# privacy-scaling-explorations/snark-verifier

Hardware: AMD Instinct MI355X
Metric: BN254 G1 MSM points/sec at 2^20 (higher is better)
Workload: dtype i32x9 (254-bit Montgomery Fq as 9 x 29-bit limbs on the integer VALU); 1 GPU; BN254 G1 Pippenger MSM, 2^20 random points/scalars per GPU, inputs resident in HBM, affine result (configs[1]); points_per_gpu=1048576, points_per_kernel_launch=1048576, window_bits=default, msms_in_flight=264

## Files before the change

snark-verifier_amd/csrc/bn254_consts.h:

```cpp
#pragma once
#define SNARKV_CURVE_NAME "bn254"
#define SNARKV_FQ_P_LIMBS { 0xd87cfd47u, 0x3c208c16u, 0x6871ca8du, 0x97816a91u, 0x8181585du, 0xb85045b6u, 0xe131a029u, 0x30644e72u }
#define SNARKV_FQ_P_INV32 0xe4866389u
#define SNARKV_FQ_ONE_MONT { 0xc58f0d9du, 0xd35d438du, 0xf5c70b3du, 0x0a78eb28u, 0x7879462cu, 0x666ea36fu, 0x9a07df2fu, 0x0e0a77c1u }
#define SNARKV_FQ_R2_MONT { 0x538afa89u, 0xf32cfc5bu, 0xd44501fbu, 0xb5e71911u, 0x0a417ff6u, 0x47ab1effu, 0xcab8351fu, 0x06d89f71u }
#define SNARKV_FQ_P_MINUS_2_LIMBS { 0xd87cfd45u, 0x3c208c16u, 0x6871ca8du, 0x97816a91u, 0x8181585du, 0xb85045b6u, 0xe131a029u, 0x30644e72u }
#define SNARKV_G1_B_MONT { 0x50ad28d7u, 0x7a17caa9u, 0xe15521b9u, 0x1f6ac17au, 0x696bd284u, 0x334bea4eu, 0xce179d8eu, 0x2a1f6744u }
#define SNARKV_FR_R_LIMBS { 0xf0000001u, 0x43e1f593u, 0x79b97091u, 0x2833e848u, 0x8181585du, 0xb85045b6u, 0xe131a029u, 0x30644e72u }
#define SNARKV_FQ29_P_LIMBS { 0x187cfd47, 0x010460b6, 0x1c72a34f, 0x02d522d0, 0x1585d978, 0x02db40c0, 0x00a6e141, 0x0e5c2634, 0x0030644e }
#define SNARKV_FQ29_NINV 0x04866389
#define SNARKV_FQ29_ONE_LIMBS { 0x157ccc21, 0x141c2758, 0x185230d3, 0x014c0419, 0x0aa36fb9, 0x1d4240ce, 0x11d54c07, 0x052ac7a8, 0x000dc836 }
#define SNARKV_FQ29_R2_LIMBS { 0x059bac10, 0x0d1503a3, 0x018016b8, 0x10ab0ca8, 0x02632639, 0x02c0169f, 0x169bfd53, 0x11869d4c, 0x002a11a6 }
#define SNARKV_FQ29_M256_IN_LIMBS { 0x13349ca1, 0x1a5d84a8, 0x0a3e5cac, 0x100249e0, 0x12b951e8, 0x0e92d304, 0x14cb95b3, 0x041b9d3d, 0x00058003 }
#define SNARKV_FQ29_M256_OUT_LIMBS { 0x058f0d9d, 0x1aea1c6e, 0x11c2cf74, 0x11d651eb, 0x1462c0a7, 0x11b7bc3c, 0x1cbd99ba, 0x183340fb, 0x000e0a77 }
#define SNARKV_FR29_P_LIMBS { 0x10000001, 0x1f0fac9f, 0x0e5c2450, 0x07d090f3, 0x1585d283, 0x02db40c0, 0x00a6e141, 0x0e5c2634, 0x0030644e }
#define SNARKV_FR29_NINV 0x0fffffff
#define SNARKV_FR29_ONE_LIMBS { 0x0fffff57, 0x1ea70ab4, 0x052c068b, 0x17504f49, 0x0aa8075b, 0x1d4240ce, 0x11d54c07, 0x052ac7a8, 0x000dc836 }
#define SNARKV_FR29_R2_LIMBS { 0x05b69bd4, 0x06170a5a, 0x020cddce, 0x1db6310b, 0x0e54d0ff, 0x1cf855e3, 0x1c15e103, 0x07d09161, 0x000a054a }
#define SNARKV_GLV_BETA29_LIMBS { 0x0a337995, 0x158d1d23, 0x189c9b98, 0x12fa4e45, 0x185faadc, 0x0176f16d, 0x0eed93ba, 0x14291140, 0x000c0afe }
#define SNARKV_GLV_A1 { 0x94d213e3u, 0x89d32568u, 0x00000000u, 0x00000000u }
#define SNARKV_GLV_NEG_B1 { 0x7d4f1128u, 0x8211bbebu, 0xeeb859fcu, 0x6f4d8248u }
#define SNARKV_GLV_A2 { 0x1221250bu, 0x0be4e154u, 0xeeb859fdu, 0x6f4d8248u }
#define SNARKV_GLV_B2 { 0x94d213e3u, 0x89d32568u, 0x00000000u, 0x00000000u }
#define SNARKV_GLV_G1 { 0x6eb9c714u, 0xc7e0b3d7u, 0xd91d232eu, 0x00000002u, 0x00000000u, 0x00000000u }
#define SNARKV_GLV_G2 { 0xa5e38cfbu, 0x391eb18du, 0x7a7bd9d4u, 0xa773d2cfu, 0x4ccef014u, 0x00000002u }
#define BN254_P_LIMBS { 0xd87cfd47u, 0x3c208c16u, 0x6871ca8du, 0x97816a91u, 0x8181585du, 0xb85045b6u, 0xe131a029u, 0x30644e72u }
#define BN254_R_LIMBS { 0xf0000001u, 0x43e1f593u, 0x79b97091u, 0x2833e848u, 0x8181585du, 0xb85045b6u, 0xe131a029u, 0x30644e72u }
#define BN254_P_INV32 0xe4866389u
#define BN254_ONE_MONT { 0xc58f0d9du, 0xd35d438du, 0xf5c70b3du, 0x0a78eb28u, 0x7879462cu, 0x666ea36fu, 0x9a07df2fu, 0x0e0a77c1u }
#define BN254_R2_MONT { 0x538afa89u, 0xf32cfc5bu, 0xd44501fbu, 0xb5e71911u, 0x0a417ff6u, 0x47ab1effu, 0xcab8351fu, 0x06d89f71u }
#define BN254_THREE_MONT { 0x50ad28d7u, 0x7a17caa9u, 0xe15521b9u, 0x1f6ac17au, 0x696bd284u, 0x334bea4eu, 0xce179d8eu, 0x2a1f6744u }
#define BN254_TWIST_B_C0_MONT { 0x77b802a8u, 0x3bf938e3u, 0x3633535du, 0x020b1b27u, 0x49755260u, 0x26b7edf0u, 0x4384a86du, 0x2514c632u }
#define BN254_TWIST_B_C1_MONT { 0xd1dcff67u, 0x38e7ecccu, 0x93ce0d3eu, 0x65f0b37du, 0x22ac00aau, 0xd749d0ddu, 0x4a688d4du, 0x0141b9ceu }
#define BN254_TWIST_3B_C0_MONT { 0xb62e0d6au, 0x3baa927cu, 0xd1b664fdu, 0xd71e7c52u, 0xd95d4664u, 0x03873e63u, 0x082ab8f4u, 0x0e75b5b1u }
#define BN254_TWIST_3B_C1_MONT { 0x7596fe35u, 0xaab7c666u, 0xbb6a27bau, 0x31d21a78u, 0x680401ffu, 0x85dd7297u, 0xdf39a7e9u, 0x03c52d6au }
#define BN254_P_MINUS_2_LIMBS { 0xd87cfd45u, 0x3c208c16u, 0x6871ca8du, 0x97816a91u, 0x8181585du, 0xb85045b6u, 0xe131a029u, 0x30644e72u }
#define BN254_P_PLUS_1_DIV_4_LIMBS { 0xb61f3f52u, 0x4f082305u, 0x5a1c72a3u, 0x65e05aa4u, 0xa0605617u, 0x6e14116du, 0xb84c680au, 0x0c19139cu }
#define BN254_X_U64 0x44e992b44a6909f1ull
#define BN254_ATE_LOOP_LO 0x9d797039be763ba8ull
#define BN254_ATE_LOOP_HI 0x1ull
#define BN254_P29_LIMBS { 0x187cfd47, 0x010460b6, 0x1c72a34f, 0x02d522d0, 0x1585d978, 0x02db40c0, 0x00a6e141, 0x0e5c2634, 0x0030644e }
#define BN254_P29_NINV 0x04866389
#define BN254_ONE29_LIMBS { 0x157ccc21, 0x141c2758, 0x185230d3, 0x014c0419, 0x0aa36fb9, 0x1d4240ce, 0x11d54c07, 0x052ac7a8, 0x000dc836 }
#define BN254_R2_29_LIMBS { 0x059bac10, 0x0d1503a3, 0x018016b8, 0x10ab0ca8, 0x02632639, 0x02c0169f, 0x169bfd53, 0x11869d4c, 0x002a11a6 }
#define BN254_THREE29_LIMBS { 0x00766463, 0x1c54760a, 0x08f6927a, 0x03e40c4d, 0x1fea4f2b, 0x17c6c26a, 0x157fe417, 0x0f8056f9, 0x002958a2 }
#define BN254_FR29_LIMBS { 0x10000001, 0x1f0fac9f, 0x0e5c2450, 0x07d090f3, 0x1585d283, 0x02db40c0, 0x00a6e141, 0x0e5c2634, 0x0030644e }
#define BN254_FR29_NINV 0x0fffffff
#define BN254_FR29_ONE_LIMBS { 0x0fffff57, 0x1ea70ab4, 0x052c068b, 0x17504f49, 0x0aa8075b, 0x1d4240ce, 0x11d54c07, 0x052ac7a8, 0x000dc836 }
#define BN254_FR29_R2_LIMBS { 0x05b69bd4, 0x06170a5a, 0x020cddce, 0x1db6310b, 0x0e54d0ff, 0x1cf855e3, 0x1c15e103, 0x07d09161, 0x000a054a }
#define BN254_FROB_GAMMA_1 { \
  { { 0x33144907u, 0xaf9ba696u, 0x87afb78au, 0xca6b1d73u, 0xf08a2087u, 0x11bded5eu, 0x1a1f3a7cu, 0x02f34d75u }, { 0x4c492d72u, 0xa222ae23u, 0x565de15bu, 0xd00f02a4u, 0x53dfc926u, 0xdc2ff3a2u, 0xb3899551u, 0x10a75716u } }, \
  { { 0x4563ab30u, 0xb5773b10u, 0xa9aa6454u, 0x347f91c8u, 0x242e0991u, 0x7a007127u, 0x118214ecu, 0x1956bcd8u }, { 0xa0aa4757u, 0x6e849f1eu, 0x89f89141u, 0xaa1c7b6du, 0xfae0ca3au, 0xb6e713cdu, 0x4e82ebc3u, 0x26694fbbu } }, \
  { { 0x2936b629u, 0xe4bbdd0cu, 0xe133bacbu, 0xbb30f162u, 0xf9645366u, 0x31a9d1b6u, 0xa500f8ddu, 0x253570beu }, { 0x5ffe77c7u, 0xa1d77ce4u, 0x7826d1dbu, 0x07affd11u, 0xbb7edc6bu, 0x6d16bd27u, 0x85defeccu, 0x2c872002u } }, \
  { { 0x843abe92u, 0x7361d77fu, 0x273411fbu, 0xa5bb2bd3u, 0x4b3e2399u, 0x9c941f31u, 0xbb9fd3ecu, 0x15df9cddu }, { 0x4bd8c949u, 0x5dddfd15u, 0xa4445b60u, 0x62cb29a5u, 0x0c7dd2b9u, 0x37bc870au, 0x3171f0fdu, 0x24830a9du } }, \
  { { 0x41690fe7u, 0xc970692fu, 0x27694b0bu, 0xe2403421u, 0x83c459e8u, 0x32bee66bu, 0x0ab08841u, 0x12aabcedu }, { 0x40aebfa9u, 0x0d485d23u, 0xab2fcc57u, 0x05193418u, 0x8a4910f5u, 0xd3b0a40bu, 0x35d2925au, 0x2f21ebb5u } }, \
}
#define BN254_FROB_GAMMA_2 { \
  { { 0x00fa1bf2u, 0xca8d8005u, 0x68b39769u, 0xf0c5d614u, 0xad0d4418u, 0x0e201271u, 0xbad856e6u, 0x04290f65u }, { 0x00000000u, 0x00000000u, 0x00000000u, 0x00000000u, 0x00000000u, 0x00000000u, 0x00000000u, 0x00000000u } }, \
  { { 0x13e80b9cu, 0x3350c88eu, 0xdb5e56b9u, 0x7dce557cu, 0xb615564au, 0x6001b4b8u, 0x020217e0u, 0x2682e617u }, { 0x00000000u, 0x00000000u, 0x00000000u, 0x00000000u, 0x00000000u, 0x00000000u, 0x00000000u, 0x00000000u } }, \
  { { 0x12edefaau, 0x68c34889u, 0x72aabf4fu, 0x8d087f68u, 0x09081231u, 0x51e1a247u, 0x4729c0fau, 0x2259d6b1u }, { 0x00000000u, 0x00000000u, 0x00000000u, 0x00000000u, 0x00000000u, 0x00000000u, 0x00000000u, 0x00000000u } }, \
  { { 0xd782e155u, 0x71930c11u, 0xffbe3323u, 0xa6bb947cu, 0xd4741444u, 0xaa303344u, 0x26594943u, 0x2c3b3f0du }, { 0x00000000u, 0x00000000u, 0x00000000u, 0x00000000u, 0x00000000u, 0x00000000u, 0x00000000u, 0x00000000u } }, \
  { { 0xc494f1abu, 0x08cfc388u, 0x8d1373d4u, 0x19b31514u, 0xcb6c0213u, 0x584e90fdu, 0xdf2f8849u, 0x09e1685bu }, { 0x00000000u, 0x00000000u, 0x00000000u, 0x00000000u, 0x00000000u, 0x00000000u, 0x00000000u, 0x00000000u } }, \
}
#define BN254_FROB_GAMMA_3 { \
  { { 0x4e46d97du, 0x36531618u, 0xd4c96d9fu, 0x0af7129eu, 0xca1009b5u, 0x659da72fu, 0x83a20d23u, 0x08116d89u }, { 0xc39c1939u, 0xb1df4af7u, 0x8a73bf7fu, 0x3d9f0287u, 0x8caf0ae0u, 0x9b222092u, 0xeff054a6u, 0x26684515u } }, \
  { { 0x16ad6badu, 0xc9af22f7u, 0x4aa662b2u, 0xb311782au, 0xe248c7f4u, 0x19eeaf64u, 0xe3439f82u, 0x20273e77u }, { 0xf7ce93acu, 0xacc02860u, 0x7ba76b4cu, 0x3933d581u, 0x446c8467u, 0x69e6188bu, 0x4417cc55u, 0x0a46036du } }, \
  { { 0xaf46471eu, 0x5764af0au, 0x873e0fc1u, 0xdc50792eu, 0x881d04f6u, 0x86a673ffu, 0x3c30a74cu, 0x0b2eddb4u }, { 0x787e8580u, 0x9a490f32u, 0xf04af8b1u, 0x8fd16d7fu, 0xc6027bf2u, 0x4b39888eu, 0x5b52a15du, 0x03dd2e70u } }, \
  { { 0x7b6762dfu, 0x448a93a5u, 0x28fdeadfu, 0xbfd62df5u, 0x0e9bd47au, 0xd858f5d0u, 0x3476ec58u, 0x06b03d4du }, { 0xbcc936d1u, 0x2b19daf4u, 0x56f4299fu, 0xa1a54e7au, 0x5adeaef1u, 0xb533eee0u, 0x84dda0b2u, 0x170c812bu } }, \
  { { 0x75cf559fu, 0xe0bc4b22u, 0xc154e60fu, 0xc238b945u, 0x929a7d5eu, 0x803982a5u, 0xf7e4a37eu, 0x15ce052du }, { 0xbf3799a7u, 0x2d28efbdu, 0x1ad60773u, 0x9b097e3cu, 0xaf4a535bu, 0x982d4113u, 0xe3056063u, 0x24e18991u } }, \
}
#define BN254_FROB29_GAMMA_1 { \
  { { 0x0a0c2399, 0x1aa2357c, 0x0149b22d, 0x0487bf1b, 0x0b89bb5e, 0x1313c7e1, 0x1d61fdb5, 0x060c56b5, 0x002e0560 }, { 0x1bc6cc33, 0x177dfb71, 0x161dd8ab, 0x0180969d, 0x058d47f5, 0x1ab975b5, 0x01c26a2d, 0x1cd88219, 0x00009b83 } }, \
  { { 0x04a59190, 0x06f504d9, 0x0bf870bb, 0x171ffd5c, 0x1ac4d17d, 0x04be36d5, 0x0bceec27, 0x1a83a513, 0x002492b3 }, { 0x11142ef1, 0x0b31acc7, 0x1d5818bc, 0x180afc17, 0x1a63177e, 0x15765b3b, 0x118f742e, 0x063a509a, 0x00135e4e } }, \
  { { 0x1b1f0678, 0x0373fb06, 0x13170fbd, 0x185d74b7, 0x0241131f, 0x16e18435, 0x1ef3b6ce, 0x01f06f02, 0x001d46bd }, { 0x19a647d5, 0x19fdefab, 0x1d925d1a, 0x0d1f6c5f, 0x08ac6cc5, 0x1fa5621a, 0x134f06fe, 0x09a72816, 0x0015871d } }, \
  { { 0x1081f85e, 0x139a3585, 0x124aed48, 0x034ce260, 0x19e166e5, 0x0b172958, 0x0d2df880, 0x0de46877, 0x00167751 }, { 0x0f616a78, 0x05940429, 0x181bb386, 0x066e257b, 0x00e66254, 0x0c12b5cd, 0x0ef6c029, 0x1c2232e3, 0x0006f9f8 } }, \
  { { 0x07461d8c, 0x0434a6b0, 0x14f8b697, 0x0b0aa80f, 0x118b92df, 0x0471333d, 0x18c6d066, 0x07d8f7b0, 0x0010a3f0 }, { 0x1eb54987, 0x08d56d1e, 0x0c80f1d8, 0x1536f380, 0x06b4b4a7, 0x082bcd3c, 0x19349170, 0x17aea9fc, 0x000817f6 } }, \
}
#define BN254_FROB29_GAMMA_2 { \
// ... 18 lines not shown
```

snark-verifier_amd/csrc/gen_consts.py:

```python
#!/usr/bin/env python3
import sys

P = 0x30644E72E131A029B85045B68181585D97816A916871CA8D3C208C16D87CFD47
R = 0x30644E72E131A029B85045B68181585D2833E84879B9709143E1F593F0000001
X = 4965661367192848881
MONT_R = 1 << 256


def generic_section(p, r, b, name):
    def lim(v):
        return ", ".join("0x%08xu" % ((v >> (32 * i)) & 0xFFFFFFFF) for i in range(8))

    def lim29(v):
        return ", ".join("0x%08x" % ((v >> (29 * i)) & ((1 << 29) - 1)) for i in range(9))

    r29 = 1 << 261
    print("// ---- field / group layer constants of %s: base field p, scalar field r, y^2 = x^3 + %d" % (name, b))
    print("#define SNARKV_CURVE_NAME \"%s\"" % name)
    print("#define SNARKV_FQ_P_LIMBS { %s }" % lim(p))
    print("#define SNARKV_FQ_P_INV32 0x%08xu  // -p^-1 mod 2^32" % ((-pow(p, -1, 1 << 32)) % (1 << 32)))
    print("#define SNARKV_FQ_ONE_MONT { %s }  // 2^256 mod p" % lim(MONT_R % p))
    print("#define SNARKV_FQ_R2_MONT { %s }  // 2^512 mod p" % lim(MONT_R * MONT_R % p))
    print("#define SNARKV_FQ_P_MINUS_2_LIMBS { %s }" % lim(p - 2))
    print("#define SNARKV_G1_B_MONT { %s }  // b * 2^256 mod p" % lim(b * MONT_R % p))
# ... 21 lines not shown
    def add(a, b):
        if a is None:
            return b
        if b is None:
            return a
        if a[0] == b[0]:
            if (a[1] + b[1]) % p == 0:
                return None
            l = 3 * a[0] * a[0] * pow(2 * a[1], -1, p) % p
        else:
            l = (b[1] - a[1]) * pow(b[0] - a[0], -1, p) % p
        x = (l * l - a[0] - b[0]) % p
        return (x, (l * (a[0] - x) - a[1]) % p)

    acc = None
    for bit in bin(k)[2:]:
        acc = add(acc, acc)
        if bit == "1":
            acc = add(acc, pt)
    return acc


def _glv_lattice(n, lam):
    import math

    rs, ts = [n, lam], [0, 1]
    sq = math.isqrt(n)
    while rs[-1] >= sq:
        q = rs[-2] // rs[-1]
        rs.append(rs[-2] - q * rs[-1])
        ts.append(ts[-2] - q * ts[-1])
    q = rs[-2] // rs[-1]
    cand = [(rs[-2], -ts[-2]), (rs[-2] - q * rs[-1], -(ts[-2] - q * ts[-1]))]
    a2, b2 = min(cand, key=lambda v: v[0] * v[0] + v[1] * v[1])
    return rs[-1], -ts[-1], a2, b2


def glv_section(p, r, gen):
    def words(v, n):
        assert 0 <= v < 1 << (32 * n)
        return ", ".join("0x%08xu" % ((v >> (32 * i)) & 0xFFFFFFFF) for i in range(n))

    def lim29(v):
        return ", ".join("0x%08x" % ((v >> (29 * i)) & ((1 << 29) - 1)) for i in range(9))

    lam = _cube_roots(r)[0]
    lg = _affine_mul(gen, lam, p)
    beta = [b for b in _cube_roots(p) if (b * gen[0] % p, gen[1]) == lg][0]
    a1, b1, a2, b2 = _glv_lattice(r, lam)
    assert a1 * b2 - a2 * b1 == r and b1 < 0 < a1 and a2 > 0 and b2 > 0
    assert (a1 + b1 * lam) % r == 0 and (a2 + b2 * lam) % r == 0
    assert a1 + a2 < (1 << 128) - (1 << 120) and -b1 + b2 < (1 << 128) - (1 << 120)
    g1, g2 = (b2 << 288) // r, ((-b1) << 288) // r
    print("// GLV: lambda^2 + lambda + 1 = 0 mod r, phi(x, y) = (beta x, y) = lambda (x, y);")
    print("// lattice (a1, b1), (a2, b2) with a + b lambda = 0 mod r, b1 < 0; g_i = floor(2^288 |b_j| / r)")
    print("// lambda = 0x%x" % lam)
    print("#define SNARKV_GLV_BETA29_LIMBS { %s }  // beta * 2^261 mod p" % lim29(beta * (1 << 261) % p))
    print("#define SNARKV_GLV_A1 { %s }  // %d bits" % (words(a1, 4), a1.bit_length()))
    print("#define SNARKV_GLV_NEG_B1 { %s }  // |b1|, %d bits" % (words(-b1, 4), (-b1).bit_length()))
    print("#define SNARKV_GLV_A2 { %s }  // %d bits" % (words(a2, 4), a2.bit_length()))
    print("#define SNARKV_GLV_B2 { %s }  // %d bits" % (words(b2, 4), b2.bit_length()))
    print("#define SNARKV_GLV_G1 { %s }  // floor(2^288 b2 / r), %d bits" % (words(g1, 6), g1.bit_length()))
    print("#define SNARKV_GLV_G2 { %s }  // floor(2^288 |b1| / r), %d bits" % (words(g2, 6), g2.bit_length()))


if len(sys.argv) > 1 and sys.argv[1] == "pallas":
    PP = 0x40000000000000000000000000000000224698FC094CF91B992D30ED00000001
    PQ = 0x40000000000000000000000000000000224698FC0994A8DD8C46EB2100000001
    assert PP == (1 << 254) + 45560315531419706090280762371685220353
    assert PQ == (1 << 254) + 45560315531506369815346746415080538113
    assert (2 * 2 - ((-1) ** 3 + 5)) % PP == 0
    print("// GENERATED by gen_consts.py pallas -- do not edit.  8x32-bit limbs little-endian; *_MONT in Montgomery")
    print("// form (R = 2^256); *29* in 9x29-bit limbs (R = 2^261).  No pairing constants: the pasta build has no KZG decider.")
    print("#pragma once")
    generic_section(PP, PQ, 5, "pallas")
    glv_section(PP, PQ, (PP - 1, 2))
    sys.exit(0)


def limbs(v):
    return ", ".join("0x%08xu" % ((v >> (32 * i)) & 0xFFFFFFFF) for i in range(8))


def mont(v):
    return v * MONT_R % P


def f2mul(a, b):
    return ((a[0] * b[0] - a[1] * b[1]) % P, (a[0] * b[1] + a[1] * b[0]) % P)


def f2pow(a, e):
    r = (1, 0)
    while e:
        if e & 1:
            r = f2mul(r, a)
        a = f2mul(a, a)
        e >>= 1
    return r


def f2inv(a):
    d = pow(a[0] * a[0] + a[1] * a[1], -1, P)
    return (a[0] * d % P, -a[1] * d % P)


XI = (9, 1)
print("// GENERATED by gen_consts.py -- do not edit.  BN254 constants, 8x32-bit limbs,")
print("// little-endian limb order; *_MONT values are in Montgomery form (R = 2^256).")
print("#pragma once")
generic_section(P, R, 3, "bn254")
glv_section(P, R, (1, 2))
print("// ---- BN254 only")
print("#define BN254_P_LIMBS { %s }" % limbs(P))
print("#define BN254_R_LIMBS { %s }" % limbs(R))
print("#define BN254_P_INV32 0x%08xu  // -p^-1 mod 2^32" % ((-pow(P, -1, 1 << 32)) % (1 << 32)))
# ... 45 lines not shown
```

snark-verifier_amd/csrc/msm_pippenger.hip:

```cpp
#include <stdlib.h>
#include <string.h>
#include <algorithm>
#include <mutex>
#include <atomic>
#include "ctx.hpp"
#include "g1_29.h"
#include "fr29.h"
#ifndef SNARKV_GLV
#define SNARKV_GLV 1
#endif
#if SNARKV_GLV
#include "glv.h"
#endif

namespace snarkv {

#ifndef SNARKV_KRUN
#define SNARKV_KRUN 128
#endif
#ifndef SNARKV_KCHUNK
#define SNARKV_KCHUNK 8
#endif
#ifndef SNARKV_TILE_THREADS
#define SNARKV_TILE_THREADS 256
#endif
#ifndef SNARKV_SCATTER_ATTR
#define SNARKV_SCATTER_ATTR __attribute__((amdgpu_waves_per_eu(5)))
#endif
#ifndef SNARKV_L2_THREADS
#define SNARKV_L2_THREADS 512
#endif
#ifndef SNARKV_LEVEL2_ATTR
#define SNARKV_LEVEL2_ATTR
#endif
#ifndef SNARKV_PREP_THREADS
#define SNARKV_PREP_THREADS SNARKV_TILE_THREADS
#endif
#ifndef SNARKV_XCD_TILES
#define SNARKV_XCD_TILES 1
#endif
#ifndef SNARKV_TILE_BASE
#define SNARKV_TILE_BASE 2048
#endif
#ifndef SNARKV_ACC_WAVES
#define SNARKV_ACC_WAVES 3
#endif
#ifndef SNARKV_BPRIO
#define SNARKV_BPRIO 3
#endif
#define SNARKV_RAISE_PRIO() __builtin_amdgcn_s_setprio(SNARKV_BPRIO)

constexpr int kHalves = SNARKV_GLV ? 2 : 1;
constexpr int kDigitWords = SNARKV_GLV ? 4 : 8;
constexpr int kDigitBits = 32 * kDigitWords;
constexpr int kRun = SNARKV_KRUN;
#ifndef SNARKV_KRUN_THROUGHPUT
#define SNARKV_KRUN_THROUGHPUT 128
#endif
constexpr int kRunThroughput = SNARKV_KRUN_THROUGHPUT;
constexpr int kChunk = SNARKV_KCHUNK;
constexpr uint32_t kSortCap = 7168;
constexpr uint32_t kSortTarget = 3072;
constexpr uint32_t kMaxKeys = 16384;

struct PipParams {
  uint32_t n;
  int c;
  int W;
  uint32_t B;
  uint32_t nb;
  int low_bits;
  uint32_t SB;
  uint32_t nkeys;
  uint32_t nblk;
  uint32_t tile;
  uint32_t mstride;
  uint32_t w0;
  uint32_t krun;
  uint32_t wper;
  uint32_t chunk_log2;
  uint32_t mont;
};

__device__ __forceinline__ uint32_t half_bits(const uint32_t (&k)[kDigitWords], int lo, int c) {
  if (lo >= kDigitBits) return 0;
  int word = lo >> 5, sh = lo & 31;
  uint32_t w0 = 0u, w1 = 0u;
#pragma unroll
  for (int i = 0; i < kDigitWords; ++i) {
    w0 = word == i ? k[i] : w0;
    if (i > 0) w1 = word == i - 1 ? k[i] : w1;
  }
  uint64_t v = ((uint64_t)w1 << 32) | w0;
  return (uint32_t)(v >> sh) & ((1u << c) - 1u);
}

template <class F>
__device__ __forceinline__ void for_each_digit(const uint32_t (&k)[kDigitWords], uint32_t sgn, const PipParams& p, F emit) {
  uint32_t carry = 0;
  for (int w = 0; w < p.W; ++w) {
    uint32_t raw = half_bits(k, w * p.c, p.c) + carry;
    uint32_t neg = raw > p.B ? 1u : 0u;
    uint32_t d = neg ? ((1u << p.c) - raw) : raw;
    carry = neg;
    if (d != 0) emit((uint32_t)w * p.SB + ((d - 1) >> p.low_bits), (uint32_t)w * p.B + d - 1, neg ^ sgn);
  }
}
template <class F>
__device__ __forceinline__ void digit_of_window(const uint32_t (&k)[kDigitWords], uint32_t sgn, const PipParams& p, int w,
                                                F emit) {
  uint32_t carry = 0;
  for (int j = w - 1; j >= 0; --j) {
    uint32_t b = half_bits(k, j * p.c, p.c);
    if (b != p.B) {
      carry = b > p.B ? 1u : 0u;
      break;
    }
  }
  uint32_t raw = half_bits(k, w * p.c, p.c) + carry;
  uint32_t neg = raw > p.B ? 1u : 0u;
  uint32_t d = neg ? ((1u << p.c) - raw) : raw;
  if (d != 0) emit((uint32_t)w * p.SB + ((d - 1) >> p.low_bits), (uint32_t)w * p.B + d - 1, neg ^ sgn);
}
__device__ __forceinline__ uint32_t load_digit_words(const uint32_t* src, uint32_t (&k)[kDigitWords]) {
#pragma unroll
  for (int j = 0; j < kDigitWords; ++j) k[j] = src[j];
#if SNARKV_GLV
  uint32_t sgn = k[3] >> 31;
  k[3] &= 0x7FFFFFFFu;
  return sgn;
#else
  return 0u;
#endif
}
__device__ __forceinline__ uint32_t load_digit_source(const uint4* __restrict__ src, size_t v, uint32_t (&k)[kDigitWords]) {
  const uint4* s = src + v * (kDigitWords / 4);
#pragma unroll
  for (int j = 0; j < kDigitWords / 4; ++j) {
    uint4 q = s[j];
    k[4 * j] = q.x;
    k[4 * j + 1] = q.y;
    k[4 * j + 2] = q.z;
    k[4 * j + 3] = q.w;
  }
#if SNARKV_GLV
  uint32_t sgn = k[3] >> 31;
  k[3] &= 0x7FFFFFFFu;
  return sgn;
#else
  return 0u;
#endif
}

__device__ __forceinline__ uint32_t xcd_tile(uint32_t b, uint32_t nblk) {
#if SNARKV_XCD_TILES
  return (nblk & 7u) == 0 ? (b & 7u) * (nblk >> 3) + (b >> 3) : b;
#else
  return b;
#endif
}

__global__ void __launch_bounds__(SNARKV_PREP_THREADS)
    k_prepare(const uint32_t* __restrict__ scalars, const uint32_t* __restrict__ points,
              G1Packed* __restrict__ pts, uint4* __restrict__ glv, PipParams p, uint32_t* __restrict__ M) {
  SNARKV_RAISE_PRIO();
  extern __shared__ uint32_t lds[];
  for (uint32_t k = threadIdx.x; k < p.nkeys; k += blockDim.x) lds[k] = 0u;
  __syncthreads();
  const uint32_t tile = xcd_tile(blockIdx.x, p.nblk);
  uint32_t lo = tile * p.tile;
  uint32_t hi = lo + p.tile < p.n ? lo + p.tile : p.n;
  for (uint32_t i = lo + threadIdx.x; i < hi; i += blockDim.x) {
    const uint4* s = reinterpret_cast<const uint4*>(points + (size_t)i * 16);
    uint32_t w[16];
#pragma unroll
    for (int j = 0; j < 4; ++j) {
      uint4 v = s[j];
      w[4 * j] = v.x;
      w[4 * j + 1] = v.y;
      w[4 * j + 2] = v.z;
      w[4 * j + 3] = v.w;
    }
    G1Affine29 a = g1a29_from_words(w, p.mont != 0);
    bool ident = g1a29_is_identity(a);
    pts[kHalves * (size_t)i] = g1a29_pack(a);
    const uint4* ks = reinterpret_cast<const uint4*>(scalars + (size_t)i * 8);
    uint4 k0 = ks[0], k1 = ks[1];
    uint32_t k[8] = {k0.x, k0.y, k0.z, k0.w, k1.x, k1.y, k1.z, k1.w}, o[8];
    if (p.mont) {
      uint32_t kc[8];
      fr_words_from_mont256(k, kc);
#pragma unroll
      for (int j = 0; j < 8; ++j) k[j] = kc[j];
    }
#if SNARKV_GLV
    constexpr int32_t bl[9] = SNARKV_GLV_BETA29_LIMBS;
    Fq29 beta;
#pragma unroll
    for (int j = 0; j < 9; ++j) beta.v[j] = bl[j];
    a.x = fq29_canon_of_product(fq29_mul(a.x, beta));
    pts[2 * (size_t)i + 1] = g1a29_pack(a);
    glv_decompose(k, o);
#else
#pragma unroll
    for (int j = 0; j < 8; ++j) o[j] = k[j];
#endif
    if (ident) {
#pragma unroll
      for (int j = 0; j < 8; ++j) o[j] = 0;
    }
    glv[2 * (size_t)i] = make_uint4(o[0], o[1], o[2], o[3]);
    glv[2 * (size_t)i + 1] = make_uint4(o[4], o[5], o[6], o[7]);
#pragma unroll
    for (int h = 0; h < kHalves; ++h) {
      uint32_t d[kDigitWords];
      uint32_t sgn = load_digit_words(o + h * kDigitWords, d);
      for_each_digit(d, sgn, p, [&](uint32_t key, uint32_t, uint32_t) { atomicAdd(&lds[key], 1u); });
    }
  }
  __syncthreads();
  for (uint32_t k = threadIdx.x; k < p.nkeys; k += blockDim.x) M[(size_t)k * p.mstride + tile] = lds[k];
  if (blockIdx.x == 0 && p.mstride > p.nblk)
    for (uint32_t k = threadIdx.x; k < p.nkeys; k += blockDim.x) M[(size_t)k * p.mstride + p.nblk] = 0u;
}

constexpr uint32_t kStageScalars = SNARKV_TILE_BASE;
constexpr uint32_t kStageItems = kStageScalars / SNARKV_TILE_THREADS;
static_assert(kStageScalars % SNARKV_TILE_THREADS == 0, "a staged tile gives every lane the same number of scalars");
__global__ void __launch_bounds__(SNARKV_TILE_THREADS) SNARKV_SCATTER_ATTR
    k_sort_scatter_staged(const uint4* __restrict__ glv, PipParams p, const uint32_t* __restrict__ M,
                          uint2* __restrict__ tmp) {
  SNARKV_RAISE_PRIO();
  extern __shared__ uint32_t lds[];
  uint32_t* gbase = lds;
  uint32_t* cnt = lds + p.SB;
  uint32_t* off = lds + 2 * p.SB;
  uint32_t* wsum = lds + 3 * p.SB;
  uint2* stage = reinterpret_cast<uint2*>(lds + 3 * p.SB + 16 + (p.SB & 1u));
  const uint32_t tid = threadIdx.x, lane = tid & 63u, wave = tid >> 6;
  const uint32_t tile = xcd_tile(blockIdx.x, p.nblk);
  const uint32_t lo = tile * kStageScalars;
  const uint32_t hi = lo + kStageScalars < p.n ? lo + kStageScalars : p.n;
  const uint32_t per = (p.SB + SNARKV_TILE_THREADS - 1) / SNARKV_TILE_THREADS;
  for (int w = 0; w < p.W; ++w) {
    for (uint32_t k = tid; k < p.SB; k += blockDim.x) {
      gbase[k] = M[((size_t)w * p.SB + k) * p.mstride + tile];
      cnt[k] = 0u;
    }
    __syncthreads();
    uint32_t ebkt[kStageItems * kHalves], erank[kStageItems * kHalves], eneg = 0u;
#pragma unroll
    for (uint32_t j = 0; j < kStageItems; ++j) {
      const uint32_t i = lo + tid + j * SNARKV_TILE_THREADS;
#pragma unroll
      for (uint32_t h = 0; h < (uint32_t)kHalves; ++h) {
        const uint32_t e = j * kHalves + h;
        ebkt[e] = 0xFFFFFFFFu;
        if (i < hi) {
          uint32_t d[kDigitWords];
          uint32_t sgn = load_digit_source(glv, (size_t)kHalves * i + h, d);
          digit_of_window(d, sgn, p, w, [&](uint32_t key, uint32_t bucket, uint32_t neg) {
            ebkt[e] = bucket - (uint32_t)w * p.B;
            eneg |= neg << e;
            erank[e] = atomicAdd(&cnt[key - (uint32_t)w * p.SB], 1u);
          });
        }
      }
    }
    __syncthreads();
    uint32_t mine = 0;
    for (uint32_t k = tid * per; k < (tid + 1) * per && k < p.SB; ++k) mine += cnt[k];
    uint32_t incl = mine;
#pragma unroll
    for (int d = 1; d < 64; d <<= 1) {
      uint32_t up = __shfl_up(incl, d, 64);
      if ((int)lane >= d) incl += up;
    }
    if (lane == 63) wsum[wave] = incl;
    __syncthreads();
    uint32_t run = incl - mine;
    for (uint32_t q = 0; q < wave; ++q) run += wsum[q];
    for (uint32_t k = tid * per; k < (tid + 1) * per && k < p.SB; ++k) {
      off[k] = run;
      run += cnt[k];
    }
    __syncthreads();
#pragma unroll
    for (uint32_t e = 0; e < kStageItems * kHalves; ++e)
      if (ebkt[e] != 0xFFFFFFFFu) {
        const uint32_t v = kHalves * (lo + tid + (e / kHalves) * SNARKV_TILE_THREADS) + (e % kHalves);
        stage[off[ebkt[e] >> p.low_bits] + erank[e]] = make_uint2(ebkt[e] + (uint32_t)w * p.B, v | (((eneg >> e) & 1u) << 31));
      }
    __syncthreads();
    const uint32_t total = off[p.SB - 1] + cnt[p.SB - 1];
    for (uint32_t idx = tid; idx < total; idx += blockDim.x) {
      const uint2 e = stage[idx];
      const uint32_t key = (e.x - (uint32_t)w * p.B) >> p.low_bits;
      tmp[gbase[key] + (idx - off[key])] = e;
    }
    __syncthreads();
  }
}

__global__ void __launch_bounds__(256) k_scan_local(uint32_t* __restrict__ data, uint32_t* __restrict__ blocksum,
                                                    uint32_t nb) {
  SNARKV_RAISE_PRIO();
  __shared__ uint32_t sh[256];
  uint32_t base = blockIdx.x * 1024 + threadIdx.x * 4;
  uint32_t v[4], s = 0;
#pragma unroll
  for (int j = 0; j < 4; ++j) {
    v[j] = (base + j < nb) ? data[base + j] : 0;
    s += v[j];
  }
  sh[threadIdx.x] = s;
  __syncthreads();
  for (uint32_t off = 1; off < 256; off <<= 1) {
    uint32_t t = (threadIdx.x >= off) ? sh[threadIdx.x - off] : 0;
    __syncthreads();
    sh[threadIdx.x] += t;
    __syncthreads();
// ... 535 lines not shown
                         void* d_out, bool partial_out, void* d_buckets_out) {
  return launch_msm_pippenger_phases(ctx, ctx->stream, PIP_PHASE_ALL, d_scalars, d_points, n, window_bits, d_out,
                                     partial_out, d_buckets_out, nullptr);
}

int launch_msm_pippenger_phases(snarkv_ctx* ctx, hipStream_t st, int phases, const void* d_scalars, const void* d_points,
                                size_t n, int window_bits, void* d_out, bool partial_out, void* d_buckets_out,
                                void* d_grid) {
  PipParams p;
  p.w0 = 0;
  p.wper = 0;
  p.chunk_log2 = (uint32_t)kLog2Chunk;
  p.mont = ctx->mont ? 1u : 0u;
  p.n = (uint32_t)n;
  p.c = window_bits > 0 ? window_bits : balance_window_bits(default_window_bits(n));
  if (p.c < 2) p.c = 2;
  if (p.c > 22) p.c = 22;
  p.W = (kDigitBits + p.c - 1) / p.c;
  p.B = 1u << (p.c - 1);
  p.nb = (uint32_t)p.W * p.B;
  int high = p.c - 1 > 10 ? p.c - 1 - 10 : 0;
  while (high < p.c - 1 && ((kHalves * n) >> (high + 1)) >= kSortTarget && ((uint64_t)p.W << (high + 1)) <= kMaxKeys) ++high;
  p.low_bits = (p.c - 1) - high;
  p.SB = p.B >> p.low_bits;
  p.nkeys = (uint32_t)p.W * p.SB;
  p.tile = SNARKV_TILE_BASE;
  static_assert(kStageItems * kHalves <= 32, "a staged lane keeps one sign bit per entry in a 32-bit word");
  const size_t lds_staged = ((size_t)3 * p.SB + 16 + (p.SB & 1u)) * 4 + (size_t)kStageScalars * kHalves * 8;
  p.nblk = (uint32_t)((n + p.tile - 1) / p.tile);
  p.mstride = p.nblk | 1u;
  uint64_t max_entries = (uint64_t)kHalves * (uint64_t)n * (uint64_t)p.W;
  if (n == 0 || max_entries >= 0xFFFFFFFFull || n >= 0x40000000ull) {
    set_last_error("pippenger: n=%zu out of range", n);
    return SNARKV_ERR_LENGTH;
  }
  if ((size_t)p.nkeys * 4 > 65536 || lds_staged > 96 * 1024) {
    set_last_error("pippenger: key table too large (nkeys=%u)", p.nkeys);
    return SNARKV_ERR_LENGTH;
  }
  p.krun = ctx->throughput_mode ? (uint32_t)kRunThroughput : latency_run_length(max_entries);
  const uint32_t max_pieces = (uint32_t)std::min<uint64_t>((uint64_t)p.nb + max_entries / p.krun, 0xFFFFFFFFull - 63);
  const uint32_t split_slots = (uint32_t)(max_entries / p.krun) + 1;
  const uint32_t nsb = (p.nb + kSchedBuckets - 1) / kSchedBuckets;
  const uint32_t hcount = sched_rows(p.krun) * nsb;
  const uint32_t hscan_blocks = (hcount + 1023) / 1024;
  uint32_t mcount = p.nkeys * p.mstride;
  uint32_t scan_blocks = (mcount + 1023) / 1024;
  uint32_t chunks_per_window = (p.B + kChunk - 1) / kChunk;
  uint32_t blocks_per_window = (chunks_per_window + 63) / 64;

  void *d_pts, *d_glv, *d_counts, *d_offsets, *d_M, *d_blocksum, *d_entries, *d_tmp, *d_pieces, *d_hist, *d_parts,
      *d_buckets, *d_wave, *d_shift, *d_misc, *d_lists;
  SNARKV_TRY(ctx_reserve(ctx, SLOT_POINTS_MONT, kHalves * n * sizeof(G1Packed), &d_pts));
  SNARKV_TRY(ctx_reserve(ctx, SLOT_GLV, n * 32, &d_glv));
  SNARKV_TRY(ctx_reserve(ctx, SLOT_COUNTS, (size_t)p.nb * 4, &d_counts));
  SNARKV_TRY(ctx_reserve(ctx, SLOT_OFFSETS, (size_t)p.nb * 4, &d_offsets));
  SNARKV_TRY(ctx_reserve(ctx, SLOT_CURSOR, (size_t)mcount * 4, &d_M));
  SNARKV_TRY(ctx_reserve(ctx, SLOT_BLOCKSUMS, (size_t)std::max(scan_blocks, hscan_blocks) * 4 + 64, &d_blocksum));
  SNARKV_TRY(ctx_reserve(ctx, SLOT_ENTRIES, max_entries * 8, &d_entries));
  SNARKV_TRY(ctx_reserve(ctx, SLOT_SORT_TMP, max_entries * 8, &d_tmp));
  SNARKV_TRY(ctx_reserve(ctx, SLOT_PIECES, (size_t)max_pieces * sizeof(uint4), &d_pieces));
  SNARKV_TRY(ctx_reserve(ctx, SLOT_PIECE_HIST, (size_t)hcount * 4, &d_hist));
  SNARKV_TRY(ctx_reserve(ctx, SLOT_SPLIT_PARTS, (size_t)split_slots * 2 * sizeof(G1Xyzz29), &d_parts));
  if (d_grid) d_buckets = d_grid;
  else SNARKV_TRY(ctx_reserve(ctx, SLOT_BUCKETS, (size_t)p.nb * sizeof(G1Xyzz29), &d_buckets));
  SNARKV_TRY(ctx_reserve(ctx, SLOT_CHUNK_PARTIALS, 2 * (size_t)blocks_per_window * p.W * sizeof(G1Xyzz29), &d_wave));
  SNARKV_TRY(ctx_reserve(ctx, SLOT_SHIFTED, (size_t)p.W * sizeof(G1Xyzz29), &d_shift));
  SNARKV_TRY(ctx_reserve(ctx, SLOT_MISC, 64, &d_misc));
  SNARKV_TRY(ctx_reserve(ctx, SLOT_FIX_LISTS, (size_t)p.nb * 3 * 4, &d_lists));
  uint32_t* d_total = (uint32_t*)d_misc;
  uint32_t* d_small = (uint32_t*)d_lists, *d_bigl = d_small + p.nb, *d_deg = d_bigl + p.nb;
  const uint32_t* d_npieces = (const uint32_t*)d_hist + (size_t)(p.krun + 1) * nsb;

  const bool tm = ctx->stage_timing && phases == PIP_PHASE_ALL;
  const bool tm_acc = ctx->stage_timing && phases == PIP_PHASE_ACC;
  int evi = 0;
#define STAGE_MARK()                                         \
  do {                                                       \
    if (tm) SNARKV_HIP(hipEventRecord(ctx->ev[evi++], st));  \
  } while (0)
  if ((tm || tm_acc) && !ctx->ev_ready) {
    for (int i = 0; i <= SNARKV_PIP_STAGES; ++i) SNARKV_HIP(hipEventCreate(&ctx->ev[i]));
    ctx->ev_ready = true;
  }
  STAGE_MARK();
  if (phases & PIP_PHASE_SORT) {
    hipLaunchKernelGGL(k_prepare, dim3(p.nblk), dim3(SNARKV_PREP_THREADS), (size_t)p.nkeys * 4, st, (const uint32_t*)d_scalars,
                       (const uint32_t*)d_points, (G1Packed*)d_pts, (uint4*)d_glv, p, (uint32_t*)d_M);
    STAGE_MARK();
    hipLaunchKernelGGL(k_scan_local, dim3(scan_blocks), dim3(256), 0, st, (uint32_t*)d_M, (uint32_t*)d_blocksum, mcount);
    hipLaunchKernelGGL(k_scan_blocksums, dim3(1), dim3(1024), 0, st, (uint32_t*)d_blocksum, scan_blocks, d_total);
    hipLaunchKernelGGL(k_scan_add, dim3(scan_blocks), dim3(256), 0, st, (uint32_t*)d_M, (const uint32_t*)d_blocksum,
                       mcount);
    STAGE_MARK();
    static std::atomic<uint64_t> attr_set{0};
    const uint64_t bit = 1ull << (ctx->device & 63);
    if (!(attr_set.load(std::memory_order_relaxed) & bit)) {
      SNARKV_HIP(hipFuncSetAttribute(reinterpret_cast<const void*>(k_sort_scatter_staged),
                                     hipFuncAttributeMaxDynamicSharedMemorySize, 96 * 1024));
      attr_set.fetch_or(bit, std::memory_order_relaxed);
    }
    hipLaunchKernelGGL(k_sort_scatter_staged, dim3(p.nblk), dim3(SNARKV_TILE_THREADS), lds_staged, st, (const uint4*)d_glv,
                       p, (const uint32_t*)d_M, (uint2*)d_tmp);
    const uint32_t nbins_l2 = 1u << p.low_bits;
    const size_t lds2 = ((size_t)nbins_l2 + SNARKV_L2_THREADS + 1) * 4 + (size_t)kSortCap * 8;
    hipLaunchKernelGGL(k_sort_level2, dim3(p.nkeys), dim3(SNARKV_L2_THREADS), lds2, st, (const uint2*)d_tmp, (const uint32_t*)d_M,
                       d_total, p, (uint2*)d_entries, (uint32_t*)d_counts, (uint32_t*)d_offsets);
// ... 157 lines not shown
```

snark-verifier_amd/csrc/pallas_consts.h:

```cpp
#pragma once
#define SNARKV_CURVE_NAME "pallas"
#define SNARKV_FQ_P_LIMBS { 0x00000001u, 0x992d30edu, 0x094cf91bu, 0x224698fcu, 0x00000000u, 0x00000000u, 0x00000000u, 0x40000000u }
#define SNARKV_FQ_P_INV32 0xffffffffu
#define SNARKV_FQ_ONE_MONT { 0xfffffffdu, 0x34786d38u, 0xe41914adu, 0x992c350bu, 0xffffffffu, 0xffffffffu, 0xffffffffu, 0x3fffffffu }
#define SNARKV_FQ_R2_MONT { 0x0000000fu, 0x8c78ecb3u, 0x8b0de0e7u, 0xd7d30dbdu, 0xc3c95d18u, 0x7797a99bu, 0x7b9cb714u, 0x096d41afu }
#define SNARKV_FQ_P_MINUS_2_LIMBS { 0xffffffffu, 0x992d30ecu, 0x094cf91bu, 0x224698fcu, 0x00000000u, 0x00000000u, 0x00000000u, 0x40000000u }
#define SNARKV_G1_B_MONT { 0xffffffedu, 0xa1a55e68u, 0x4f4982f3u, 0x74c2a54bu, 0xfffffffdu, 0xffffffffu, 0xffffffffu, 0x3fffffffu }
#define SNARKV_FR_R_LIMBS { 0x00000001u, 0x8c46eb21u, 0x0994a8ddu, 0x224698fcu, 0x00000000u, 0x00000000u, 0x00000000u, 0x40000000u }
#define SNARKV_FQ29_P_LIMBS { 0x00000001, 0x09698768, 0x133e46e6, 0x0d31f812, 0x00000224, 0x00000000, 0x00000000, 0x00000000, 0x00400000 }
#define SNARKV_FQ29_NINV 0x1fffffff
#define SNARKV_FQ29_ONE_LIMBS { 0x1fffff81, 0x14a5d367, 0x141ad3c0, 0x1435eec5, 0x1ffeefef, 0x1fffffff, 0x1fffffff, 0x1fffffff, 0x003fffff }
#define SNARKV_FQ29_R2_LIMBS { 0x00003b6a, 0x19c10910, 0x1a6a0188, 0x12a4fd88, 0x0634b36d, 0x178792ba, 0x07797a99, 0x1dce5b8a, 0x003506bd }
#define SNARKV_FQ29_M256_IN_LIMBS { 0x1ffff001, 0x10f30767, 0x0ecfe231, 0x0db0ce73, 0x1fddbb8b, 0x1fffffff, 0x1fffffff, 0x1fffffff, 0x003fffff }
#define SNARKV_FQ29_M256_OUT_LIMBS { 0x1ffffffd, 0x03c369c7, 0x06452b4d, 0x186a17c8, 0x1ffff992, 0x1fffffff, 0x1fffffff, 0x1fffffff, 0x003fffff }
#define SNARKV_FR29_P_LIMBS { 0x00000001, 0x02375908, 0x052a3763, 0x0d31f813, 0x00000224, 0x00000000, 0x00000000, 0x00000000, 0x00400000 }
#define SNARKV_FR29_NINV 0x1fffffff
#define SNARKV_FR29_ONE_LIMBS { 0x1fffff81, 0x068ad507, 0x100e85da, 0x1435ee7e, 0x1ffeefef, 0x1fffffff, 0x1fffffff, 0x1fffffff, 0x003fffff }
#define SNARKV_FR29_R2_LIMBS { 0x00003b6a, 0x02b1b550, 0x1027888a, 0x1ea4ed96, 0x0418ad7a, 0x000999eb, 0x17fae231, 0x1e67ed54, 0x003506bd }
#define SNARKV_GLV_BETA29_LIMBS { 0x1342a796, 0x03fdac51, 0x054dab11, 0x05b221a6, 0x0ccd27ac, 0x15cc87a4, 0x1b1533b6, 0x169e85e1, 0x003b0093 }
#define SNARKV_GLV_A1 { 0x00000001u, 0x7fcae1c7u, 0x40f04915u, 0x49e69d16u }
#define SNARKV_GLV_NEG_B1 { 0x00000000u, 0x8cb12793u, 0x40a89953u, 0x49e69d16u }
#define SNARKV_GLV_A2 { 0x00000000u, 0x8cb12793u, 0x40a89953u, 0x49e69d16u }
#define SNARKV_GLV_B2 { 0x00000001u, 0x0c7c095au, 0x8198e269u, 0x93cd3a2cu }
#define SNARKV_GLV_G1 { 0xc35fbd4du, 0x00000002u, 0x31f02568u, 0x066389a4u, 0x4f34e8b2u, 0x00000002u }
#define SNARKV_GLV_G2 { 0x61afdea6u, 0xffffffffu, 0x32c49e4bu, 0x02a2654eu, 0x279a7459u, 0x00000001u }
```

Before: 809.9 million points/s.

## Store carry-resolved signed digits so scatter reads each window field directly

The counting pass now resolves the signed-digit carries once per scalar half and writes the carry-resolved halves back to the GLV buffer. The sign goes either into bit 127 or into a separate ballot-built sign bitmap when the resolved value needs all 128 bits, as on Pallas. The per-window scatter pass then extracts each window's field with a direct bit slice instead of scanning lower windows to recover the carry. This removes the per-window backward carry search and the branchy word selection, at the cost of slightly more work and stores in the count kernel plus extra sign-map bookkeeping.

```diff
diff --git a/snark-verifier_amd/csrc/bn254_consts.h b/snark-verifier_amd/csrc/bn254_consts.h
--- a/snark-verifier_amd/csrc/bn254_consts.h
+++ b/snark-verifier_amd/csrc/bn254_consts.h
@@ -24,6 +24,8 @@
 #define SNARKV_GLV_B2 { 0x94d213e3u, 0x89d32568u, 0x00000000u, 0x00000000u }
 #define SNARKV_GLV_G1 { 0x6eb9c714u, 0xc7e0b3d7u, 0xd91d232eu, 0x00000002u, 0x00000000u, 0x00000000u }
 #define SNARKV_GLV_G2 { 0xa5e38cfbu, 0x391eb18du, 0x7a7bd9d4u, 0xa773d2cfu, 0x4ccef014u, 0x00000002u }
+#define SNARKV_GLV_HALF_MAX { 0xb8e79e27u, 0x068a19ddu, 0x932f8d91u, 0x37a6c124u }
+#define SNARKV_GLV_RESOLVED_BITS 127
 #define BN254_P_LIMBS { 0xd87cfd47u, 0x3c208c16u, 0x6871ca8du, 0x97816a91u, 0x8181585du, 0xb85045b6u, 0xe131a029u, 0x30644e72u }
 #define BN254_R_LIMBS { 0xf0000001u, 0x43e1f593u, 0x79b97091u, 0x2833e848u, 0x8181585du, 0xb85045b6u, 0xe131a029u, 0x30644e72u }
 #define BN254_P_INV32 0xe4866389u
diff --git a/snark-verifier_amd/csrc/digits.h b/snark-verifier_amd/csrc/digits.h
--- /dev/null
+++ b/snark-verifier_amd/csrc/digits.h
@@ -0,0 +1,83 @@
+#pragma once
+#include "fq.h"
+
+namespace snarkv {
+
+constexpr bool kDigitSignInWord = SNARKV_GLV_RESOLVED_BITS <= 127;
+static_assert(SNARKV_GLV_RESOLVED_BITS <= 128, "a carry-resolved GLV half fits its 128-bit slot");
+
+SNARKV_HD bool digit_of_field(uint32_t t, int c, uint32_t& d, uint32_t& neg) {
+  const uint32_t B = 1u << (c - 1);
+  neg = t > B ? 1u : 0u;
+  d = neg ? (1u << c) - t : t;
+  return t != 0u;
+}
+
+template <int C, int NW, class F>
+SNARKV_HD void digits_resolve_aligned(const uint32_t (&k)[NW], uint32_t (&out)[NW], F field) {
+  static_assert(32 % C == 0, "aligned fields tile a word");
+  constexpr uint32_t mask = (1u << C) - 1u, B = 1u << (C - 1);
+  uint32_t carry = 0u;
+#pragma unroll
+  for (int j = 0; j < NW; ++j) {
+    uint32_t o = 0u;
+#pragma unroll
+    for (int f = 0; f < 32 / C; ++f) {
+      const uint32_t raw = ((k[j] >> (f * C)) & mask) + carry;
+      carry = raw > B ? 1u : 0u;
+      const uint32_t t = raw & mask;
+      o |= t << (f * C);
+      field(j * (32 / C) + f, t);
+    }
+    out[j] = o;
+  }
+}
+
+template <int NW, class F>
+SNARKV_HD void digits_resolve(const uint32_t (&k)[NW], int c, uint32_t (&out)[NW], F field) {
+  const uint32_t mask = (1u << c) - 1u, B = 1u << (c - 1);
+  uint64_t in = 0, res = 0;
+  int nin = 0, nres = 0, w = 0;
+  uint32_t carry = 0u;
+#pragma unroll
+  for (int j = 0; j < NW; ++j) {
+    in |= (uint64_t)k[j] << nin;
+    nin += 32;
+    while (nin >= c) {
+      const uint32_t raw = ((uint32_t)in & mask) + carry;
+      carry = raw > B ? 1u : 0u;
+      const uint32_t t = raw & mask;
+      res |= (uint64_t)t << nres;
+      nres += c;
+      in >>= c;
+      nin -= c;
+      field(w++, t);
+    }
+    if (j > 0) {
+      out[j - 1] = (uint32_t)res;
+      res >>= 32;
+      nres -= 32;
+    }
+  }
+  if (nin > 0) {
+    const uint32_t t = (uint32_t)in + carry;
+    res |= (uint64_t)t << nres;
+    field(w, t);
+  }
+  out[NW - 1] = (uint32_t)res;
+}
+
+SNARKV_HD uint32_t digits_field(const uint32_t* K, int nwords, int c, int w, uint32_t top_mask) {
+  const int lo = w * c, word = lo >> 5, sh = lo & 31;
+  uint32_t v = K[word];
+  if (word == nwords - 1) v &= top_mask;
+  uint32_t t = v >> sh;
+  if (sh + c > 32 && word + 1 < nwords) {
+    uint32_t v1 = K[word + 1];
+    if (word + 1 == nwords - 1) v1 &= top_mask;
+    t |= v1 << (32 - sh);
+  }
+  return t & ((1u << c) - 1u);
+}
+
+}
diff --git a/snark-verifier_amd/csrc/gen_consts.py b/snark-verifier_amd/csrc/gen_consts.py
--- a/snark-verifier_amd/csrc/gen_consts.py
+++ b/snark-verifier_amd/csrc/gen_consts.py
@@ -97,6 +97,14 @@
     assert (a1 + b1 * lam) % r == 0 and (a2 + b2 * lam) % r == 0
     assert a1 + a2 < (1 << 128) - (1 << 120) and -b1 + b2 < (1 << 128) - (1 << 120)
     g1, g2 = (b2 << 288) // r, ((-b1) << 288) // r
+    kmax = (max(a1 + a2, -b1 + b2) * ((1 << 33) + 1) + (1 << 34) - 1) >> 34
+    resolved_bits = 0
+    for c in range(2, 23):
+        s = ((128 + c - 1) // c - 1) * c
+        top = (kmax >> s) + 1
+        assert top <= 1 << (c - 1)
+        resolved_bits = max(resolved_bits, (top << s).bit_length())
+    assert resolved_bits <= 128
     print("// GLV: lambda^2 + lambda + 1 = 0 mod r, phi(x, y) = (beta x, y) = lambda (x, y);")
     print("// lattice (a1, b1), (a2, b2) with a + b lambda = 0 mod r, b1 < 0; g_i = floor(2^288 |b_j| / r)")
     print("// lambda = 0x%x" % lam)
@@ -107,6 +115,10 @@
     print("#define SNARKV_GLV_B2 { %s }  // %d bits" % (words(b2, 4), b2.bit_length()))
     print("#define SNARKV_GLV_G1 { %s }  // floor(2^288 b2 / r), %d bits" % (words(g1, 6), g1.bit_length()))
     print("#define SNARKV_GLV_G2 { %s }  // floor(2^288 |b1| / r), %d bits" % (words(g2, 6), g2.bit_length()))
+    print("#define SNARKV_GLV_HALF_MAX { %s }  // |k_i| <= ceil((1/2 + 2^-34) max(a1 + a2, |b1| + b2)), %d bits"
+          % (words(kmax, 4), kmax.bit_length()))
+    print("#define SNARKV_GLV_RESOLVED_BITS %d  // bits of the largest carry-resolved half, c = 2 .. 22 (digits.h): "
+          "bit 127 %s" % (resolved_bits, "is free for the sign" if resolved_bits <= 127 else "is NOT free for a sign"))
 
 
 if len(sys.argv) > 1 and sys.argv[1] == "pallas":
diff --git a/snark-verifier_amd/csrc/msm_pippenger.hip b/snark-verifier_amd/csrc/msm_pippenger.hip
--- a/snark-verifier_amd/csrc/msm_pippenger.hip
+++ b/snark-verifier_amd/csrc/msm_pippenger.hip
@@ -6,6 +6,7 @@
 #include "ctx.hpp"
 #include "g1_29.h"
 #include "fr29.h"
+#include "digits.h"
 #ifndef SNARKV_GLV
 #define SNARKV_GLV 1
 #endif
@@ -82,45 +83,15 @@
   uint32_t mont;
 };
 
-__device__ __forceinline__ uint32_t half_bits(const uint32_t (&k)[kDigitWords], int lo, int c) {
-  if (lo >= kDigitBits) return 0;
-  int word = lo >> 5, sh = lo & 31;
-  uint32_t w0 = 0u, w1 = 0u;
-#pragma unroll
-  for (int i = 0; i < kDigitWords; ++i) {
-    w0 = word == i ? k[i] : w0;
-    if (i > 0) w1 = word == i - 1 ? k[i] : w1;
-  }
-  uint64_t v = ((uint64_t)w1 << 32) | w0;
-  return (uint32_t)(v >> sh) & ((1u << c) - 1u);
-}
-
-template <class F>
-__device__ __forceinline__ void for_each_digit(const uint32_t (&k)[kDigitWords], uint32_t sgn, const PipParams& p, F emit) {
-  uint32_t carry = 0;
-  for (int w = 0; w < p.W; ++w) {
-    uint32_t raw = half_bits(k, w * p.c, p.c) + carry;
-    uint32_t neg = raw > p.B ? 1u : 0u;
-    uint32_t d = neg ? ((1u << p.c) - raw) : raw;
-    carry = neg;
-    if (d != 0) emit((uint32_t)w * p.SB + ((d - 1) >> p.low_bits), (uint32_t)w * p.B + d - 1, neg ^ sgn);
-  }
-}
-template <class F>
-__device__ __forceinline__ void digit_of_window(const uint32_t (&k)[kDigitWords], uint32_t sgn, const PipParams& p, int w,
-                                                F emit) {
-  uint32_t carry = 0;
-  for (int j = w - 1; j >= 0; --j) {
-    uint32_t b = half_bits(k, j * p.c, p.c);
-    if (b != p.B) {
-      carry = b > p.B ? 1u : 0u;
-      break;
-    }
-  }
-  uint32_t raw = half_bits(k, w * p.c, p.c) + carry;
-  uint32_t neg = raw > p.B ? 1u : 0u;
-  uint32_t d = neg ? ((1u << p.c) - raw) : raw;
-  if (d != 0) emit((uint32_t)w * p.SB + ((d - 1) >> p.low_bits), (uint32_t)w * p.B + d - 1, neg ^ sgn);
+constexpr bool kHasSign = SNARKV_GLV != 0;
+constexpr bool kSignBit = kHasSign && kDigitSignInWord;
+constexpr bool kSignMap = kHasSign && !kDigitSignInWord;
+constexpr uint32_t kTopMask = kSignBit ? 0x7FFFFFFFu : 0xFFFFFFFFu;
+constexpr int kSourceQuads = kHalves * kDigitWords / 4;
+__host__ __device__ inline size_t sign_map_words(size_t n) { return kSignMap ? (size_t)kHalves * ((n + 63) / 64) : 0; }
+__device__ __forceinline__ void count_field(uint32_t* lds, const PipParams& p, int c, int w, uint32_t t) {
+  uint32_t d, neg;
+  if (digit_of_field(t, c, d, neg)) atomicAdd(&lds[(uint32_t)w * p.SB + ((d - 1) >> p.low_bits)], 1u);
 }
 __device__ __forceinline__ uint32_t load_digit_words(const uint32_t* src, uint32_t (&k)[kDigitWords]) {
 #pragma unroll
@@ -133,24 +104,6 @@
   return 0u;
 #endif
 }
-__device__ __forceinline__ uint32_t load_digit_source(const uint4* __restrict__ src, size_t v, uint32_t (&k)[kDigitWords]) {
-  const uint4* s = src + v * (kDigitWords / 4);
-#pragma unroll
-  for (int j = 0; j < kDigitWords / 4; ++j) {
-    uint4 q = s[j];
-    k[4 * j] = q.x;
-    k[4 * j + 1] = q.y;
-    k[4 * j + 2] = q.z;
-    k[4 * j + 3] = q.w;
-  }
-#if SNARKV_GLV
-  uint32_t sgn = k[3] >> 31;
-  k[3] &= 0x7FFFFFFFu;
-  return sgn;
-#else
-  return 0u;
-#endif
-}
 
 __device__ __forceinline__ uint32_t xcd_tile(uint32_t b, uint32_t nblk) {
 #if SNARKV_XCD_TILES
@@ -170,6 +123,7 @@
   const uint32_t tile = xcd_tile(blockIdx.x, p.nblk);
   uint32_t lo = tile * p.tile;
   uint32_t hi = lo + p.tile < p.n ? lo + p.tile : p.n;
+  unsigned long long* signs = reinterpret_cast<unsigned long long*>(glv + (size_t)p.n * kSourceQuads);
   for (uint32_t i = lo + threadIdx.x; i < hi; i += blockDim.x) {
     const uint4* s = reinterpret_cast<const uint4*>(points + (size_t)i * 16);
     uint32_t w[16];
@@ -209,13 +163,24 @@
 #pragma unroll
       for (int j = 0; j < 8; ++j) o[j] = 0;
     }
-    glv[2 * (size_t)i] = make_uint4(o[0], o[1], o[2], o[3]);
-    glv[2 * (size_t)i + 1] = make_uint4(o[4], o[5], o[6], o[7]);
 #pragma unroll
     for (int h = 0; h < kHalves; ++h) {
-      uint32_t d[kDigitWords];
-      uint32_t sgn = load_digit_words(o + h * kDigitWords, d);
-      for_each_digit(d, sgn, p, [&](uint32_t key, uint32_t, uint32_t) { atomicAdd(&lds[key], 1u); });
+      uint32_t d[kDigitWords], r[kDigitWords];
+      const uint32_t sgn = load_digit_words(o + h * kDigitWords, d);
+      if (p.c == 16)
+        digits_resolve_aligned<16>(d, r, [&](int w, uint32_t t) { count_field(lds, p, 16, w, t); });
+      else if (p.c == 8)
+        digits_resolve_aligned<8>(d, r, [&](int w, uint32_t t) { count_field(lds, p, 8, w, t); });
+      else
+        digits_resolve(d, p.c, r, [&](int w, uint32_t t) { count_field(lds, p, p.c, w, t); });
+      if (kSignBit) r[kDigitWords - 1] |= sgn << 31;
+      if (kSignMap) {
+        const unsigned long long m = __ballot(sgn != 0u);
+        if ((threadIdx.x & 63u) == 0u) signs[(size_t)h * ((p.n + 63u) / 64u) + (i >> 6)] = m;
+      }
+#pragma unroll
+      for (int q = 0; q < kDigitWords / 4; ++q)
+        glv[(kHalves * (size_t)i + h) * (kDigitWords / 4) + q] = make_uint4(r[4 * q], r[4 * q + 1], r[4 * q + 2], r[4 * q + 3]);
     }
   }
   __syncthreads();
@@ -242,6 +207,19 @@
   const uint32_t lo = tile * kStageScalars;
   const uint32_t hi = lo + kStageScalars < p.n ? lo + kStageScalars : p.n;
   const uint32_t per = (p.SB + SNARKV_TILE_THREADS - 1) / SNARKV_TILE_THREADS;
+  const uint32_t* K = reinterpret_cast<const uint32_t*>(glv);
+  uint32_t hsgn = 0u;
+  if (kHasSign) {
+    const unsigned long long* signs = reinterpret_cast<const unsigned long long*>(glv + (size_t)p.n * kSourceQuads);
+#pragma unroll
+    for (uint32_t e = 0; e < kStageItems * kHalves; ++e) {
+      const uint32_t i = lo + tid + (e / kHalves) * SNARKV_TILE_THREADS, h = e % kHalves;
+      if (i < hi)
+        hsgn |= (kSignBit ? K[((size_t)kHalves * i + h) * kDigitWords + kDigitWords - 1] >> 31
+                          : (uint32_t)(signs[(size_t)h * ((p.n + 63u) / 64u) + (i >> 6)] >> (i & 63u)) & 1u)
+                << e;
+    }
+  }
   for (int w = 0; w < p.W; ++w) {
     for (uint32_t k = tid; k < p.SB; k += blockDim.x) {
       gbase[k] = M[((size_t)w * p.SB + k) * p.mstride + tile];
@@ -257,16 +235,17 @@
         const uint32_t e = j * kHalves + h;
         ebkt[e] = 0xFFFFFFFFu;
         if (i < hi) {
-          uint32_t d[kDigitWords];
-          uint32_t sgn = load_digit_source(glv, (size_t)kHalves * i + h, d);
-          digit_of_window(d, sgn, p, w, [&](uint32_t key, uint32_t bucket, uint32_t neg) {
-            ebkt[e] = bucket - (uint32_t)w * p.B;
+          const uint32_t t = digits_field(K + ((size_t)kHalves * i + h) * kDigitWords, kDigitWords, p.c, w, kTopMask);
+          uint32_t d, neg;
+          if (digit_of_field(t, p.c, d, neg)) {
+            ebkt[e] = d - 1;
             eneg |= neg << e;
-            erank[e] = atomicAdd(&cnt[key - (uint32_t)w * p.SB], 1u);
-          });
+            erank[e] = atomicAdd(&cnt[(d - 1) >> p.low_bits], 1u);
+          }
         }
       }
     }
+    eneg ^= hsgn;
     __syncthreads();
     uint32_t mine = 0;
     for (uint32_t k = tid * per; k < (tid + 1) * per && k < p.SB; ++k) mine += cnt[k];
@@ -908,7 +887,7 @@
   void *d_pts, *d_glv, *d_counts, *d_offsets, *d_M, *d_blocksum, *d_entries, *d_tmp, *d_pieces, *d_hist, *d_parts,
       *d_buckets, *d_wave, *d_shift, *d_misc, *d_lists;
   SNARKV_TRY(ctx_reserve(ctx, SLOT_POINTS_MONT, kHalves * n * sizeof(G1Packed), &d_pts));
-  SNARKV_TRY(ctx_reserve(ctx, SLOT_GLV, n * 32, &d_glv));
+  SNARKV_TRY(ctx_reserve(ctx, SLOT_GLV, n * 32 + sign_map_words(n) * 8, &d_glv));
   SNARKV_TRY(ctx_reserve(ctx, SLOT_COUNTS, (size_t)p.nb * 4, &d_counts));
   SNARKV_TRY(ctx_reserve(ctx, SLOT_OFFSETS, (size_t)p.nb * 4, &d_offsets));
   SNARKV_TRY(ctx_reserve(ctx, SLOT_CURSOR, (size_t)mcount * 4, &d_M));
diff --git a/snark-verifier_amd/csrc/pallas_consts.h b/snark-verifier_amd/csrc/pallas_consts.h
--- a/snark-verifier_amd/csrc/pallas_consts.h
+++ b/snark-verifier_amd/csrc/pallas_consts.h
@@ -24,3 +24,5 @@
 #define SNARKV_GLV_B2 { 0x00000001u, 0x0c7c095au, 0x8198e269u, 0x93cd3a2cu }
 #define SNARKV_GLV_G1 { 0xc35fbd4du, 0x00000002u, 0x31f02568u, 0x066389a4u, 0x4f34e8b2u, 0x00000002u }
 #define SNARKV_GLV_G2 { 0x61afdea6u, 0xffffffffu, 0x32c49e4bu, 0x02a2654eu, 0x279a7459u, 0x00000001u }
+#define SNARKV_GLV_HALF_MAX { 0xa64b4c3cu, 0xfd26f765u, 0x988db3aeu, 0x6ed9eba1u }
+#define SNARKV_GLV_RESOLVED_BITS 128
```

Measured after the change: 807.7 million points/s. No clear change (-0.3%).
